# iqbal-lab-org/make_prg

Hardware: AMD Instinct MI355X
Metric: MSAs/sec (from_msa, whole node) on 30k-gene pan-genome (higher is better)
Workload: dtype u8 (+f64 KMeans)

## Files before the change

### include/mprg.h

```cpp
#ifndef MPRG_H
#define MPRG_H
#include <stdint.h>

#ifdef __cplusplus
extern "C" {
#endif

enum {
  MPRG_V_RM_BASE = 0, MPRG_V_CM_BASE = 1, MPRG_V_PITCH_C = 2, MPRG_V_PITCH_S = 3, MPRG_V_ROWS_OFF = 4,
  MPRG_V_N_ROWS = 5, MPRG_V_COL0 = 6, MPRG_V_N_COLS = 7, MPRG_V_COL_OFF = 8, MPRG_V_ROW_OFF = 9,
  MPRG_V_AUX0 = 10, MPRG_V_AUX1 = 11, MPRG_VIEW_FIELDS = 12
};
enum { MPRG_CODE_GAP = 4, MPRG_CODE_N = 11, MPRG_N_CODES = 12 };
enum { MPRG_IV_MATCH = 0, MPRG_IV_NONMATCH = 1 ,
       MPRG_IV_PURE = 2  };
enum { MPRG_ST_PARTITION_ERROR = 1, MPRG_ST_ALL_N_SLICE = 2,
       MPRG_ST_BAD_LAUNCH = 4  };
enum { MPRG_KM_RELOCATED = 1 ,
       MPRG_KM_UNSUPPORTED = 2  };

const char *mprg_version(void);
const char *mprg_last_error(void);
int mprg_device_cus(void);

// ... 53 lines not shown
int mprg_kmeans_fit_split(const int64_t *prob, const int32_t *kinfo, const int32_t *fit_list, int n_fits, int n_init,
                          const double *uniforms_dev, const double *xcounts, double *ws, int32_t *labels, double *km_info,
                          int32_t *km_status, void *stream);
int mprg_kmeans_prepare_big(const int64_t *prob, const double *xcounts, double *ws, const int32_t *list, int n_list, uint8_t *xbytes,
                            int with_tables, void *stream);
int mprg_kmeans_fit_wide(const int64_t *prob, const int32_t *kinfo, const int32_t *fit_list, int n_fits, int n_init,
                         const double *uniforms_dev, const double *xcounts, double *ws, int32_t *labels, double *km_info,
                         int32_t *km_status, const uint8_t *xbytes, void *stream);
int mprg_kmeans_wave_class(int64_t D, int64_t V, int k);
int mprg_kmeans_small_class(int64_t D, int64_t V, int k, int n_init);
int mprg_kmeans_fit_small(const int64_t *prob, const int32_t *kinfo, const int32_t *fit_list, int n_fits, int small_class, int n_init,
                          const double *uniforms_dev, const double *xcounts, double *ws, int32_t *labels, double *km_info,
                          int32_t *km_status, void *stream);
int mprg_kmeans_lds_class(int64_t D, int64_t V, int k, int n_init);
int mprg_kmeans_fit_lds(const int64_t *prob, const int32_t *kinfo, const int32_t *fit_list, int n_fits, int lds_class, int n_init,
                        const double *uniforms_dev, const double *xcounts, double *ws, int32_t *labels, double *km_info,
                        int32_t *km_status, void *stream);
int mprg_kmeans_fit_wave(const int64_t *prob, const int32_t *kinfo, const int32_t *fit_list, int n_fits, int lds_class, int n_init,
                         const double *uniforms_dev, const double *xcounts, double *ws, int32_t *labels, double *km_info,
                         int32_t *km_status, void *stream);
void mprg_random_sample_host(uint32_t seed, int n, double *out_host);

enum { MPRG_CF_TILE = 256, MPRG_CF_TILE_BIG = 32, MPRG_CF_ROWS = 1024, MPRG_CF_WIDE = 512, MPRG_CF_ROWS_WIDE = 16 };
int mprg_cluster_further(const uint8_t *arena, const int64_t *views, const int32_t *rowidx, const int64_t *prob,
                         int n_probs, int k, const int32_t *d_of_row, const int32_t *labels, int32_t *assign,
                         const int32_t *work_cols, int n_work_cols, const int32_t *work_rows, int n_work_rows,
                         int32_t *scratch, int32_t *out_further, const double *km_info, const uint8_t *gcodes, const int32_t *kinfo,
                         void *stream);
int mprg_cluster_further_bounded(const uint8_t *arena, const int64_t *views, const int32_t *rowidx, const int64_t *prob,
                                 int n_probs, int k, const int32_t *d_of_row, const int32_t *labels, int32_t *assign,
                                 const int32_t *work_cols, int n_work_cols, const int32_t *work_rows, int n_work_rows,
                                 int32_t *scratch, int32_t *out_further, const double *km_info, const uint8_t *gcodes, const int32_t *kinfo,
                                 long long max_rows, void *stream);

enum { MPRG_LOOP_GENERAL = 1, MPRG_LOOP_SMALL_LOW = 2, MPRG_LOOP_SMALL_HIGH = 4, MPRG_LOOP_SKIP_SMALL = 8,
       MPRG_LOOP_LDS = 16 ,
       MPRG_LOOP_SKIP_LDS = 32  };
int mprg_cluster_loop(const int64_t *views, const int64_t *prob, int n_probs, int n_init, const double *uniforms_dev,
                      const int32_t *uniform_offsets_host, const double *xcounts, double *ws, const int32_t *d_of_row,
                      const uint8_t *gcodes, int32_t *scratch, int32_t *labels, int32_t *assign, double *km_info, int32_t *km_status,
                      int32_t *num_clusters, int32_t *active, int64_t *stats, int forms, void *stream);

int mprg_kmeans_speculative_kinfo(const int64_t *prob, int n_probs, int n_init, int mode, const int32_t *uniform_offsets_host,
                                  long long labels_per_k, int32_t *kinfo_out, const double *ws, void *stream);

int mprg_split_children(const int64_t *views, const int32_t *rowidx, const int64_t *prob, int n_probs,
// ... 212 lines not shown
```

### make_prg_amd/csrc/k_cluster.inc

```
#define CF_TILE 256
#define CF_TILE_BIG 32
#define CF_ROWS 1024
static_assert(CF_TILE == MPRG_CF_TILE && CF_TILE_BIG == MPRG_CF_TILE_BIG && CF_ROWS == MPRG_CF_ROWS, "include/mprg.h documents the tiles");
MPRG_DEV long long cf_col_tiles(long long n_cols, long long n_rows) {
  const long long tw = n_rows > CF_ROWS ? CF_TILE_BIG : CF_TILE;
  return (n_cols + tw - 1) / tw;
}
#ifndef CFH_WIDE
#define CFH_WIDE MPRG_CF_WIDE
#endif
#define CFH_G 16
#define CFH_ROWS_WIDE 16
static_assert(CFH_ROWS_WIDE == MPRG_CF_ROWS_WIDE, "include/mprg.h documents the chunks");
MPRG_DEV int cf_chunk_rows(long long n_cols, long long n_rows) { return (n_cols >= CFH_WIDE && n_rows > CF_ROWS) ? CFH_ROWS_WIDE : CF_TILE; }
MPRG_DEV long long cf_row_chunks(long long n_cols, long long n_rows) { const int ch = cf_chunk_rows(n_cols, n_rows); return (n_rows + ch - 1) / ch; }
#define CFO_THREADS 128
#define CFO_POOL 8192
MPRG_DEV long long cf_lds_bytes(long long S, long long n, long long k) {
  const long long cp = (n + 3) & ~3LL;
  return ((S + 3) & ~3LL) + ((2 * S + 3) & ~3LL) + k * cp + S * cp;
}
MPRG_DEV bool cf_one_fits(long long S, long long n, long long k) { return S >= 1 && S < 65536 && n >= 1 && cf_lds_bytes(S, n, k) <= CFO_POOL; }
#ifndef CF_THREADS
#define CF_THREADS 128
#endif
KERNEL(k_cluster_majority, const uint8_t *arena, const int64_t *views, const int32_t *rowidx, const int64_t *prob_all,
       const int32_t *work, int k, const int32_t *d_of_row_all, const int32_t *labels_all, int32_t *assign_all,
       const double *km_info, int32_t *scratch_all, const uint8_t *gcodes_all, const int32_t *kinfo, int one_form, DsCount dc) {
  DS_GUARD(dc, 1);
  const int32_t *wk = work + 2 * (long long)BLOCK_ID;
  if (kinfo && kinfo[5 * (long long)wk[0] + 1] == 0) return;
  const int64_t *P = prob_all + (long long)wk[0] * PF;
  const ViewD d = load_view(views, (int)P[0]);
  if (one_form && cf_one_fits(d.n_rows, d.n_cols, k)) return;
  const int n = d.n_cols, S = d.n_rows, D = (int)P[1], tile = S > CF_ROWS ? CF_TILE_BIG : CF_TILE, c0 = wk[1] * tile;
  const int32_t *dor = d_of_row_all + d.row_off;
  const int32_t *labels = labels_all ? labels_all + P[10] : nullptr;
  uint8_t *maj = (uint8_t *)(scratch_all + d.col_off * 3);
  SHARED(uint32_t, cnt, 12 * CF_THREADS);
  SHARED(int32_t, first, 12 * CF_THREADS);
  if (wk[1] == 0 && labels && assign_all && (!km_info || km_info[8 * (long long)wk[0] + 3] >= (double)k)) {
    PAR_FOR(q, D) { assign_all[P[10] + q] = labels[q]; }
  }
  if (S > CF_ROWS) return;
  SHARED(int32_t, mrk, 2 * CF_ROWS);
  int32_t *mrow = mrk, *mkey = mrk + CF_ROWS;
  SHARED(int, coff, 16);
  SHARED(int, cfill, 16);
  PAR_FOR(q, 16) { coff[q] = 0; }
  BARRIER();
  PAR_FOR(i, S) {
    const int dd = dor[i];
    if (dd < 0) continue;
    const int cl = labels ? labels[dd] : 0;
    if (cl >= 0 && cl < k) ATOMIC_ADD(coff + cl + 1, 1);
  }
  BARRIER();
// ... 32 lines not shown
        for (int q = 0; q < 8; ++q) x[q] = col[(long long)mrow[m + q] * cpitch] & 15u;
#pragma unroll
        for (int q = 0; q < 8; ++q) CF_COUNT(x[q], mkey[m + q]);
      }
      for (; m < m1; ++m) { const unsigned x = col[(long long)mrow[m] * cpitch] & 15u; CF_COUNT(x, mkey[m]); }
    }
    if (slices > 1) BARRIER();
    if (live && sl == 0) {
      int best = 0; uint32_t best_n = 0; int32_t best_key = 0x7fffffff;
      for (int s = 0; s < 12; ++s) {
        uint32_t a = cnt[s * CF_THREADS + t]; int32_t key = first[s * CF_THREADS + t];
        for (int o = 1; o < slices; ++o) {
          a += cnt[s * CF_THREADS + t + o * n_items];
          const int32_t ko = first[s * CF_THREADS + t + o * n_items];
          if (ko < key) key = ko;
        }
        if (s == 0 || a > best_n || (a == best_n && key < best_key)) { best = s; best_n = a; best_key = key; }
      }
      maj[(long long)cl * n + c] = (uint8_t)best;
    }
  }
#undef CF_COUNT
}

#define CFB_THREADS 1024
KERNEL(k_cluster_majority_big, const uint8_t *arena, const int64_t *views, const int32_t *rowidx, const int64_t *prob_all,
       const int32_t *work, int k, const int32_t *d_of_row_all, const int32_t *labels_all, int32_t *scratch_all,
       const uint8_t *gcodes_all, const int32_t *kinfo, DsCount dc) {
  DS_GUARD(dc, 1);
  const int32_t *wk = work + 2 * (long long)BLOCK_ID;
  if (kinfo && kinfo[5 * (long long)wk[0] + 1] == 0) return;
  const int64_t *P = prob_all + (long long)wk[0] * PF;
  const ViewD d = load_view(views, (int)P[0]);
  const int n = d.n_cols, S = d.n_rows, c0 = wk[1] * CF_TILE_BIG;
  if (S <= CF_ROWS) return;
  const int32_t *dor = d_of_row_all + d.row_off;
  const int32_t *labels = labels_all ? labels_all + P[10] : nullptr;
  uint8_t *maj = (uint8_t *)(scratch_all + d.col_off * 3);
  __shared__ uint32_t cnt[KM_KMAX * CF_TILE_BIG * 12];
  __shared__ unsigned long long key[KM_KMAX * CF_TILE_BIG * 12];
  const int ncols = n - c0 < CF_TILE_BIG ? n - c0 : CF_TILE_BIG;
  PAR_FOR(e, k * CF_TILE_BIG * 12) { cnt[e] = 0; key[e] = ~0ULL; }
  BARRIER();
  const int t = (int)threadIdx.x, cg = t % (CF_TILE_BIG / 4), sl = t / (CF_TILE_BIG / 4), slices = N_THREADS / (CF_TILE_BIG / 4), cb = 4 * cg;
  if (cb < ncols && sl < slices) {
    const uint8_t *col = gcodes_all ? gcodes_all + d.aux0 + c0 + cb : arena + d.rm + d.col0 + c0 + cb;
    const long long cpitch = gcodes_all ? u_pitch(n) : d.pitchC;
    const int per = (S + slices - 1) / slices, i0 = sl * per, i1 = (sl + 1) * per < S ? (sl + 1) * per : S;
#define CFB_ROW(w_, dd_, i_, cl_) do {                                                                                                \
      const unsigned long long key_ = ((unsigned long long)(uint32_t)(dd_) << 32) | (uint32_t)(i_);                                   \
      _Pragma("unroll") for (int u_ = 0; u_ < 4; ++u_) {                                                                              \
        const unsigned x_ = ((w_) >> (8 * u_)) & 15u;                                                                                 \
        if (cb + u_ < ncols && x_ < 12) {                                                                                             \
          const int at_ = (((cl_) * CF_TILE_BIG + cb + u_) * 12) + (int)x_;                                                           \
// ... 15 lines not shown
    }
    for (; i < i1; ++i) {
      const int dd = dor[i];
      if (dd < 0) continue;
      const int cl = labels ? labels[dd] : 0;
      if (cl < 0 || cl >= k) continue;
      uint32_t w;
      __builtin_memcpy(&w, col + (long long)(gcodes_all ? i : view_row(d, rowidx, i)) * cpitch, 4);
      CFB_ROW(w, dd, i, cl);
    }
#undef CFB_ROW
  }
  BARRIER();
  PAR_FOR(e, k * ncols) {
    const int cl = (int)e / ncols, c = (int)e % ncols;
    const uint32_t *cn = cnt + (cl * CF_TILE_BIG + c) * 12;
    const unsigned long long *ky = key + (cl * CF_TILE_BIG + c) * 12;
    int best = 0; uint32_t best_n = 0; unsigned long long best_key = ~0ULL;
    for (int s = 0; s < 12; ++s)
      if (s == 0 || cn[s] > best_n || (cn[s] == best_n && ky[s] < best_key)) { best = s; best_n = cn[s]; best_key = ky[s]; }
    maj[(long long)cl * n + c0 + c] = (uint8_t)best;
  }
}

KERNEL(k_cluster_hamming, const uint8_t *arena, const int64_t *views, const int32_t *rowidx, const int64_t *prob_all,
       const int32_t *work, const int32_t *d_of_row_all, const int32_t *labels_all, const int32_t *scratch_all,
       int32_t *out_further, const uint8_t *gcodes_all, const int32_t *kinfo, int one_form_k, DsCount dc) {
  DS_GUARD(dc, 1);
  const int32_t *wk = work + 2 * (long long)BLOCK_ID;
  if (kinfo && kinfo[5 * (long long)wk[0] + 1] == 0) return;
  const int64_t *P = prob_all + (long long)wk[0] * PF;
  const ViewD d = load_view(views, (int)P[0]);
  if (one_form_k && cf_one_fits(d.n_rows, d.n_cols, one_form_k)) return;
  const int n = d.n_cols, S = d.n_rows, chunk = cf_chunk_rows(n, S), r0 = wk[1] * chunk;
  const int32_t *dor = d_of_row_all + d.row_off;
  const int32_t *labels = labels_all ? labels_all + P[10] : nullptr;
  const uint8_t *maj = (const uint8_t *)(scratch_all + d.col_off * 3);
  const int thresh = n < 5 ? 1 : (int)(0.2 * (double)n);
  if (gcodes_all && n >= CFH_WIDE && (N_THREADS % CFH_G) == 0) {
    const int gl = (int)threadIdx.x % CFH_G, rows_per_pass = N_THREADS / CFH_G;
    for (int ib = r0; ib < r0 + chunk && ib < S; ib += rows_per_pass) {
      const int i = ib + (int)threadIdx.x / CFH_G;
      int stop = (gl == 0) ? *(volatile int32_t *)(out_further + wk[0]) : 0;
      stop = __shfl(stop, 0, CFH_G);
      const int dd = (i < S && i < r0 + chunk) ? dor[i] : -1;
      const bool active = !stop && dd >= 0;
      const int cl = (active && labels) ? labels[dd] : 0;
      const uint8_t *m = maj + (long long)cl * n;
      const uint8_t *grow = gcodes_all + d.aux0 + (long long)(active ? i : 0) * u_pitch(n);
      int dist = 0;
      bool far = false;
      for (int c0 = 0; c0 < n; c0 += 8 * CFH_G * 4) {
        if (active && !far) {
#pragma unroll
          for (int q = 0; q < 4; ++q) {
            const int c = c0 + (q * CFH_G + gl) * 8;
// ... 29 lines not shown
    int dist = 0;
    if (gcodes_all) {
      const uint8_t *grow = gcodes_all + d.aux0 + (long long)i * u_pitch(n);
      for (int c = 0; c < n && dist <= thresh; c += 8) {
        uint64_t x, y;
        __builtin_memcpy(&x, grow + c, 8);
        __builtin_memcpy(&y, m + c, 8);
        uint64_t v = (x ^ y) & 0x0f0f0f0f0f0f0f0fULL;
        if (c + 8 > n) v &= 0xffffffffffffffffULL >> (8 * (c + 8 - n));
        const uint64_t nz = (((v & 0x7f7f7f7f7f7f7f7fULL) + 0x7f7f7f7f7f7f7f7fULL) | v) & 0x8080808080808080ULL;
        dist += __popcll(nz);
      }
    } else
    for (int c = 0; c < n && dist <= thresh; c += 8) {
      unsigned x[8], y[8];
#pragma unroll
      for (int q = 0; q < 8; ++q) { const int cc = c + q < n ? c + q : n - 1; x[q] = cell_t(arena, d, row, cc); y[q] = m[cc]; }
#pragma unroll
      for (int q = 0; q < 8; ++q) dist += (c + q < n && x[q] != y[q]) ? 1 : 0;
    }
    if (dist > thresh) out_further[wk[0]] = 1;
  }
}

#define SC_RANKS 1024
#define SC_THREADS 64
MPRG_DEV int sc_rank(const int32_t *dor, const int32_t *sor, const int32_t *assign, int kfin, int c0, int i) {
  const int c = dor[i] >= 0 ? assign[dor[i]] : kfin + sor[i];
  return c == c0 ? 0 : (c < c0 ? c + 1 : c);
}
KERNEL(k_split_children, const int64_t *views, const int32_t *rowidx, const int64_t *prob_all, const int64_t *sp_all,
       const int32_t *d_of_row_all, const int32_t *s_of_row_all, const int32_t *assign_all, int32_t *pool_out,
       int32_t *child_sizes, DsCount dc) {
  DS_GUARD(dc, 1);
  const int64_t *P = prob_all + (long long)BLOCK_ID * PF;
  const int64_t *sp = sp_all + 3 * (long long)BLOCK_ID;
  const ViewD d = load_view(views, (int)P[0]);
  const int S = d.n_rows, kfin = (int)sp[0];
  const int32_t *dor = d_of_row_all + d.row_off, *sor = s_of_row_all + d.row_off, *assign = assign_all + P[10];
  int32_t *out = pool_out + sp[1], *sizes = child_sizes + sp[2];
  const int lane = wave_lane();
  SHARED(int, off_s, SC_RANKS);
  int nshort = 0;
  for (int i = lane; i < S; i += WAVE) nshort = sor[i] + 1 > nshort ? sor[i] + 1 : nshort;
#pragma unroll
  for (int dlt = 32; dlt >= 1; dlt >>= 1) { const int y = __shfl_xor(nshort, dlt); nshort = y > nshort ? y : nshort; }
// ... 50 lines not shown
```

### make_prg_amd/csrc/k_kloop.inc

```

#ifndef KL_CF_FN
#define KL_CF_FN MPRG_DEV
#endif
#ifdef MPRG_TEST_CF_GLOBAL
#define KL_CF_IN_LDS(fits) false
#else
#define KL_CF_IN_LDS(fits) (fits)
#endif
#define KL_CF_FIELD_BITS 32
MPRG_DEV int cf_row_cluster(int i, const uint8_t *mlab_s, const int32_t *dor, const int32_t *labels) {
  if (mlab_s) return mlab_s[i];
  const int dd = dor[i];
  return dd < 0 ? 255 : labels[dd];
}
template <int FB> struct CfWords {
  static constexpr int PER = 64 / FB, W = 12 / PER;
  unsigned long long w[W];
  MPRG_DEVM void clear() {
#pragma unroll
    for (int q = 0; q < W; ++q) w[q] = 0;
  }
  MPRG_DEVM void add(unsigned x) {
    const unsigned long long inc = x < 12 ? 1ull << (FB * (x % PER)) : 0ull;
    const unsigned sel = x / PER;
// ... 91 lines not shown
    const uint8_t *m = maj + (long long)cl * n;
    const uint8_t *grow = G + (long long)i * cpitch;
    int dist = 0;
#pragma nounroll
    for (int c = 0; c < n && dist <= thresh; c += 8) {
      uint64_t x, y;
      __builtin_memcpy(&x, grow + c, 8);
      __builtin_memcpy(&y, m + c, 8);
      uint64_t v = (x ^ y) & 0x0f0f0f0f0f0f0f0fULL;
      if (c + 8 > n) v &= 0xffffffffffffffffULL >> (8 * (c + 8 - n));
      const uint64_t nz = (((v & 0x7f7f7f7f7f7f7f7fULL) + 0x7f7f7f7f7f7f7f7fULL) | v) & 0x8080808080808080ULL;
      dist += __popcll(nz);
    }
    if (dist > thresh) flag_s[0] = 1;
  }
  BARRIER();
  const bool further = flag_s[0] != 0;
  BARRIER();
  return further;
}

template <bool OPT = false>
MPRG_DEV bool cf_problem_lds(const int S, const int n, const int D, const int k, const int32_t *dor, const int32_t *labels, int32_t *assign,
                             const uint8_t *G, uint8_t *pool, int *flag_s) {
  typedef CfWords<16> Words;
  const int cpitch = u_pitch(n), cp = (n + 3) & ~3, cw4 = cp >> 2;
  uint8_t *mlab = pool;
  uint16_t *dk = (uint16_t *)(pool + ((S + 3) & ~3));
  uint8_t *majs = (uint8_t *)dk + ((2 * S + 3) & ~3);
  uint8_t *cells = majs + k * cp;
  if (!OPT || assign) { PAR_FOR(q, D) { assign[q] = labels[q]; } }
  PAR_FOR(i, S) { const int dd = dor[i]; mlab[i] = dd < 0 ? (uint8_t)255 : ((OPT && !labels) ? (uint8_t)0 : (uint8_t)labels[dd]); dk[i] = (uint16_t)dd; }
  PAR_FOR(e, S * cw4) {
    const int i = (int)((unsigned)e / (unsigned)cw4), w = (int)((unsigned)e % (unsigned)cw4);
    *(uint32_t *)(cells + i * cp + 4 * w) = *(const uint32_t *)(G + (long long)i * cpitch + 4 * w) & 0x0f0f0f0fu;
  }
  ONE_THREAD { flag_s[0] = 0; }
  BARRIER();
  PAR_FOR(item, k * n) {
    const int cl = (int)((unsigned)item / (unsigned)n), c = (int)((unsigned)item % (unsigned)n);
    Words cw;
    cw.clear();
    const uint8_t *col = cells + c;
    int i = 0;
    for (; i + 4 <= S; i += 4) {
      unsigned rc[4], x[4];
#pragma unroll
      for (int q = 0; q < 4; ++q) { rc[q] = mlab[i + q]; x[q] = col[(i + q) * cp]; }
#pragma unroll
      for (int q = 0; q < 4; ++q) cw.add(rc[q] == (unsigned)cl ? x[q] : 15u);
    }
    for (; i < S; ++i) cw.add(mlab[i] == cl ? (unsigned)col[i * cp] : 15u);
    unsigned long long best_n = 0;
#pragma unroll
    for (int s_ = 0; s_ < 12; ++s_) { const unsigned long long a = cw.count(s_); best_n = a > best_n ? a : best_n; }
    unsigned tied = 0;
#pragma unroll
    for (int s_ = 0; s_ < 12; ++s_) if (cw.count(s_) == best_n) tied |= 1u << s_;
    int best = __ffs(tied) - 1;
    if (best_n > 0 && (tied & (tied - 1))) {
      int best_key = 0x7fffffff;
// ... 185 lines not shown
      atomicAdd((unsigned long long *)stats + KL_ST_FITS, (unsigned long long)st_i[2]);
      atomicAdd((double *)stats + KL_ST_BYTES_SMALL, st_d[0]);
      if (st_d[1] != 0) atomicAdd((double *)stats + KL_ST_CF, st_d[1]);
      if (st_i[3]) stats[KL_ST_BAD] = 1;
    }
  }
}
__attribute__((amdgpu_flat_work_group_size(64, 1024), amdgpu_waves_per_eu(KM_WAVES, KM_WAVES))) __global__ void k_cluster_loop_lds(
    const int64_t *prob_all, int n_init, const double *uniforms_all, KlUoff uoff, const double *xcounts, double *ws_all,
    const int64_t *views, const int32_t *d_of_row_all, const uint8_t *gcodes_all, int32_t *scratch_all, int32_t *labels_all,
    int32_t *assign_all, double *km_info, int32_t *km_status, int32_t *num_clusters, int32_t *active, int64_t *stats, int cls, int lds_bytes,
    DsCount dc) {
  DS_GUARD(dc, 1);
  HIP_DYNAMIC_SHARED(uint8_t, pool)
  const int b = BLOCK_ID;
  if (!active[b]) return;
  const int64_t *P = prob_all + (long long)b * PF;
  const int c = kml_class_ws(P[1], P[7], num_clusters[b] + 1, n_init, true, ws_all + P[9]);
  if (c < 0 || c > cls) return;
  kll_problem(b, prob_all, n_init, uniforms_all, uoff, xcounts, ws_all, views, d_of_row_all, gcodes_all, scratch_all, labels_all, assign_all, km_info,
              km_status, num_clusters, active, stats, pool, lds_bytes, cls);
}

KERNEL(k_cluster_further_one, const int64_t *views, const int64_t *prob_all, int n_probs, int k, const int32_t *d_of_row_all,
       const int32_t *labels_all, int32_t *assign_all, const double *km_info, int32_t *out_further, const uint8_t *gcodes_all,
       const int32_t *kinfo, DsCount dc) {
  DS_GUARD(dc, 1);
  const int b = BLOCK_ID;
  if (kinfo && kinfo[5 * (long long)b + 1] == 0) return;
  const int64_t *P = prob_all + (long long)b * PF;
  const ViewD d = load_view(views, (int)P[0]);
  if (!cf_one_fits(d.n_rows, d.n_cols, k)) return;
  __shared__ __attribute__((aligned(16))) uint8_t pool[CFO_POOL];
  SHARED(int, flag, 1);
  const int32_t *labels = labels_all ? labels_all + P[10] : nullptr;
  int32_t *assign = (labels && assign_all && (!km_info || km_info[8 * (long long)b + 3] >= (double)k)) ? assign_all + P[10] : nullptr;
  const bool further = cf_problem_lds<true>(d.n_rows, d.n_cols, (int)P[1], k, d_of_row_all + d.row_off, labels, assign, gcodes_all + d.aux0, pool, flag);
  ONE_THREAD { out_further[b] = further ? 1 : 0; }
}
```

### make_prg_amd/csrc/mprg_api.hip

```cpp
#include "mprg_platform.h"
#include "../../include/mprg.h"
#include <stdio.h>
#include <initializer_list>
#include <string.h>

#include "k_ingest.inc"
#include "k_columns.inc"
#include "k_partition.inc"
#include "k_rows.inc"
#include "k_kmer.inc"
#include "k_kmeans.inc"
#include "k_kmeans_lds.inc"
#include "k_cluster.inc"
#include "k_kloop.inc"
#include "k_emit.inc"
#include "k_forest.inc"
#include "k_align.inc"
#include "k_star.inc"
#include "k_refine.inc"
#include "k_prog.inc"
#include "k_prog_band.inc"
#include "host_encoders.inc"
#include "host_batch.inc"

static thread_local char g_err[512] = "";
static int fail(const char *what) { snprintf(g_err, sizeof g_err, "%s", what); return -1; }

// ... 11 lines not shown
  const char *e = getenv(name);
  const int v = e ? atoi(e) : dflt;
  return (v >= 64 && v <= hi && v % 64 == 0) ? v : dflt;
}
static const int g_pf_threads = env_threads("MPRG_PF_THREADS", BLOCK_VIEW);
static const int g_dd_threads = env_threads("MPRG_DD_THREADS", BLOCK_VIEW, 512);
static const int g_km_threads = env_threads("MPRG_KM_THREADS", 256);
static const int g_km_wide_threads = env_threads("MPRG_KM_WIDE_THREADS", 1024);
static const int g_kp_threads = env_threads("MPRG_KP_THREADS", 0);
static const int g_kp_tiled = [] { const char *e = getenv("MPRG_KP_TILED"); return (e && atoi(e) == 0) ? 0 : 1; }();
static const int g_kpw_split = [] { const char *e = getenv("MPRG_KPW_SPLIT"); return (e && atoi(e) == 0) ? 0 : 1; }();
static const int g_kms_threads = env_threads("MPRG_KMS_THREADS", 128, 128);
static const int g_kml_flags = [] { const char *e = getenv("MPRG_KML_FLAGS"); return e ? (atoi(e) & 0x7f) : 0; }();
static const int g_kml_threads[KML_CLASSES] = {env_threads("MPRG_KML_THREADS0", 128, 256), env_threads("MPRG_KML_THREADS1", 128, 256),
                                               env_threads("MPRG_KML_THREADS2", 256, 1024), env_threads("MPRG_KML_THREADS3", 256, 1024),
                                               env_threads("MPRG_KML_THREADS4", 512, 1024), env_threads("MPRG_KML_THREADS5", 1024, 1024)};
template <class K> static int kml_raise_lds(K kernel, bool *raised, const char *what) {
  if (*raised) return 0;
  if (hipFuncSetAttribute((const void *)kernel, hipFuncAttributeMaxDynamicSharedMemorySize, KML_C5) != hipSuccess) return fail(what);
  *raised = true;
  return 0;
}
static const int g_cf_one = [] { const char *e = getenv("MPRG_CF_ONE"); return (e && atoi(e) == 0) ? 0 : 1; }();
static const int g_pw_wave = [] { const char *e = getenv("MPRG_WAVE_VIEWS"); return (e && atoi(e) == 0) ? 0 : 1; }();
static const int g_row_views = [] { const char *e = getenv("MPRG_ROW_VIEWS"); return (e && atoi(e) == 0) ? 0 : 1; }();
#define RV_THREADS 128
#define RV_THREADS_S 64

extern "C" {

#ifndef MPRG_BUILD_TAG
#define MPRG_BUILD_TAG "hip gfx950"
#endif
const char *mprg_version(void) { return "mprg 0.2 (" MPRG_BUILD_TAG ")"; }
const char *mprg_last_error(void) { return g_err; }

int mprg_device_cus(void) {
  int dev = 0; hipDeviceProp_t p;
  if (hipGetDevice(&dev) != hipSuccess || hipGetDeviceProperties(&p, dev) != hipSuccess) return fail("no HIP device");
  return p.multiProcessorCount;
}

int mprg_ingest(const uint8_t *raw, const int64_t *msa_table, int n_msas, int64_t n_tiles, const uint8_t *n_replacement,
                uint8_t *arena, int64_t arena_bytes, int32_t *status, void *stream) {
  if (n_msas <= 0) return 0;
  if (hipMemsetAsync(arena, 15, (size_t)arena_bytes, (hipStream_t)stream) != hipSuccess) return fail("memset");
// ... 318 lines not shown
int mprg_kmeans_lds_class(int64_t D, int64_t V, int k, int n_init) { return kml_class(D, V, k, n_init); }

int mprg_kmeans_fit_lds(const int64_t *prob, const int32_t *kinfo, const int32_t *fit_list, int n_fits, int lds_class, int n_init,
                        const double *uniforms_dev, const double *xcounts, double *ws, int32_t *labels, double *km_info,
                        int32_t *km_status, void *stream) {
  if (n_fits <= 0) return 0;
  if (n_init < 1 || n_init > KML_RMAX) return fail("mprg_kmeans_fit_lds: n_init must be 1..10");
  if (lds_class < 0 || lds_class >= KML_CLASSES) return fail("mprg_kmeans_fit_lds: lds_class must be 0..5 (mprg_kmeans_lds_class)");
  const int bytes = kml_class_bytes(lds_class);
  static bool raised = false;
  if (bytes > 56 * 1024 && kml_raise_lds(k_kmeans_fit_lds, &raised, "mprg_kmeans_fit_lds: the device refuses the LDS of the largest class") != 0) return -1;
  LAUNCH_LDS(k_kmeans_fit_lds, n_fits, g_kml_threads[lds_class], bytes, stream, prob, kinfo, fit_list, n_init, uniforms_dev, xcounts, ws, labels,
             km_info, km_status, bytes | (g_kml_flags << 24));
  return check_launch("k_kmeans_fit_lds");
}

int mprg_kmeans_select(const int64_t *prob, const int32_t *kinfo, int n_fits, int n_init, const double *xcounts,
                       double *ws, int32_t *labels, double *km_info, void *stream) {
  if (n_fits <= 0) return 0;
  LAUNCH(k_kmeans_select, n_fits, 256, stream, prob, kinfo, n_init, xcounts, ws, labels, km_info);
  return check_launch("k_kmeans_select");
}

static int d_cluster_further(const uint8_t *arena, const int64_t *views, const int32_t *rowidx, const int64_t *prob,
                             int n_probs, int k, const int32_t *d_of_row, const int32_t *labels, int32_t *assign,
                             const int32_t *work_cols, int n_work_cols, const int32_t *work_rows, int n_work_rows,
                             int32_t *scratch, int32_t *out_further, const double *km_info, const uint8_t *gcodes, const int32_t *kinfo,
                             void *stream, DsCount dc_cols, DsCount dc_rows, DsCount dc_probs, long long max_rows = 0);
int mprg_cluster_further(const uint8_t *arena, const int64_t *views, const int32_t *rowidx, const int64_t *prob,
                         int n_probs, int k, const int32_t *d_of_row, const int32_t *labels, int32_t *assign,
                         const int32_t *work_cols, int n_work_cols, const int32_t *work_rows, int n_work_rows,
                         int32_t *scratch, int32_t *out_further, const double *km_info, const uint8_t *gcodes, const int32_t *kinfo,
                         void *stream) {
  return d_cluster_further(arena, views, rowidx, prob, n_probs, k, d_of_row, labels, assign, work_cols, n_work_cols, work_rows, n_work_rows,
                           scratch, out_further, km_info, gcodes, kinfo, stream, DS_HOST, DS_HOST, DS_HOST);
}
int mprg_cluster_further_bounded(const uint8_t *arena, const int64_t *views, const int32_t *rowidx, const int64_t *prob,
                                 int n_probs, int k, const int32_t *d_of_row, const int32_t *labels, int32_t *assign,
                                 const int32_t *work_cols, int n_work_cols, const int32_t *work_rows, int n_work_rows,
                                 int32_t *scratch, int32_t *out_further, const double *km_info, const uint8_t *gcodes, const int32_t *kinfo,
                                 long long max_rows, void *stream) {
  return d_cluster_further(arena, views, rowidx, prob, n_probs, k, d_of_row, labels, assign, work_cols, n_work_cols, work_rows, n_work_rows,
                           scratch, out_further, km_info, gcodes, kinfo, stream, DS_HOST, DS_HOST, DS_HOST, max_rows);
}
static int d_cluster_further(const uint8_t *arena, const int64_t *views, const int32_t *rowidx, const int64_t *prob,
                             int n_probs, int k, const int32_t *d_of_row, const int32_t *labels, int32_t *assign,
                             const int32_t *work_cols, int n_work_cols, const int32_t *work_rows, int n_work_rows,
                             int32_t *scratch, int32_t *out_further, const double *km_info, const uint8_t *gcodes, const int32_t *kinfo,
                             void *stream, DsCount dc_cols, DsCount dc_rows, DsCount dc_probs, long long max_rows) {
  if (n_probs <= 0) return 0;
  if (k < 1 || k > KM_KMAX) return fail("mprg_cluster_further: k out of range");
  if (hipMemsetAsync(out_further, 0, sizeof(int32_t) * n_probs, (hipStream_t)stream) != hipSuccess) return fail("memset");
  const int one = (g_cf_one && gcodes) ? 1 : 0;
  if (one) LAUNCH(k_cluster_further_one, n_probs, CFO_THREADS, stream, views, prob, n_probs, k, d_of_row, labels, assign, km_info, out_further, gcodes,
                  kinfo, dc_probs);
  const int big = (max_rows <= 0 || max_rows > CF_ROWS) ? 1 : 0;
  LAUNCH(k_cluster_majority, n_work_cols, CF_THREADS, stream, arena, views, rowidx, prob, work_cols, k, d_of_row, labels,
         assign, km_info, scratch, gcodes, kinfo, one, dc_cols);
  if (big) LAUNCH(k_cluster_majority_big, n_work_cols, CFB_THREADS, stream, arena, views, rowidx, prob, work_cols, k, d_of_row, labels,
                  scratch, gcodes, kinfo, dc_cols);
  LAUNCH(k_cluster_hamming, n_work_rows, CF_TILE, stream, arena, views, rowidx, prob, work_rows, d_of_row, labels,
         (const int32_t *)scratch, out_further, gcodes, kinfo, one ? k : 0, dc_rows);
  return check_launch("k_cluster_further");
}

static int d_cluster_loop(const int64_t *views, const int64_t *prob, int n_probs, int n_init, const double *uniforms_dev,
                          const int32_t *uniform_offsets_host, const double *xcounts, double *ws, const int32_t *d_of_row,
                          const uint8_t *gcodes, int32_t *scratch, int32_t *labels, int32_t *assign, double *km_info, int32_t *km_status,
                          int32_t *num_clusters, int32_t *active, int64_t *stats, int forms, void *stream, DsCount dc);
int mprg_cluster_loop(const int64_t *views, const int64_t *prob, int n_probs, int n_init, const double *uniforms_dev,
                      const int32_t *uniform_offsets_host, const double *xcounts, double *ws, const int32_t *d_of_row,
                      const uint8_t *gcodes, int32_t *scratch, int32_t *labels, int32_t *assign, double *km_info, int32_t *km_status,
                      int32_t *num_clusters, int32_t *active, int64_t *stats, int forms, void *stream) {
  return d_cluster_loop(views, prob, n_probs, n_init, uniforms_dev, uniform_offsets_host, xcounts, ws, d_of_row, gcodes, scratch, labels, assign,
                        km_info, km_status, num_clusters, active, stats, forms, stream, DS_HOST);
}
static int d_cluster_loop(const int64_t *views, const int64_t *prob, int n_probs, int n_init, const double *uniforms_dev,
                          const int32_t *uniform_offsets_host, const double *xcounts, double *ws, const int32_t *d_of_row,
                          const uint8_t *gcodes, int32_t *scratch, int32_t *labels, int32_t *assign, double *km_info, int32_t *km_status,
                          int32_t *num_clusters, int32_t *active, int64_t *stats, int forms, void *stream, DsCount dc) {
  if (n_probs <= 0) return 0;
  if (n_init < 1 || n_init > KM_RMAX) return fail("n_init must be 1..16");
  if (!gcodes || !uniform_offsets_host || !stats) return fail("mprg_cluster_loop: gcodes, uniform_offsets_host and stats are required");
  if (!(forms & (7 | MPRG_LOOP_LDS))) return fail("mprg_cluster_loop: forms must name a workgroup form (MPRG_LOOP_*)");
  KlUoff uoff;
// ... 638 lines not shown
```

Baseline: 133,900.

## Bin cluster-further problems into LDS size classes with persistent compacted launches

Problems are first compacted on the device into four lists by shared-memory footprint (8K to 64K pools), and the single-block LDS path then runs once per class with per-class thread counts in persistent grid-stride loops. Problems that fit no class go to a rest list, which is handled by persistent majority/hamming kernels that ballot-scan the work list. Before, every problem got its own block and the fallback kernels early-exited. The LDS path also gains multi-slice column counting and vectorised 16-byte cell loads. The cost is an extra compaction kernel, a cached per-stream list buffer guarded by a mutex, and a raised dynamic LDS limit, which may lower occupancy for the larger classes.

After: 134,200 (median of 3 runs). About the same (+0.2%).

```diff
diff --git a/include/mprg.h b/include/mprg.h
--- a/include/mprg.h
+++ b/include/mprg.h
@@ -99,6 +99,7 @@
 void mprg_random_sample_host(uint32_t seed, int n, double *out_host);
 
 enum { MPRG_CF_TILE = 256, MPRG_CF_TILE_BIG = 32, MPRG_CF_ROWS = 1024, MPRG_CF_WIDE = 512, MPRG_CF_ROWS_WIDE = 16 };
+enum { MPRG_CF_CLASSES = 4, MPRG_CF_POOL0 = 8192 };
 int mprg_cluster_further(const uint8_t *arena, const int64_t *views, const int32_t *rowidx, const int64_t *prob,
                          int n_probs, int k, const int32_t *d_of_row, const int32_t *labels, int32_t *assign,
                          const int32_t *work_cols, int n_work_cols, const int32_t *work_rows, int n_work_rows,
diff --git a/make_prg_amd/csrc/k_cluster.inc b/make_prg_amd/csrc/k_cluster.inc
--- a/make_prg_amd/csrc/k_cluster.inc
+++ b/make_prg_amd/csrc/k_cluster.inc
@@ -14,25 +14,63 @@
 static_assert(CFH_ROWS_WIDE == MPRG_CF_ROWS_WIDE, "include/mprg.h documents the chunks");
 MPRG_DEV int cf_chunk_rows(long long n_cols, long long n_rows) { return (n_cols >= CFH_WIDE && n_rows > CF_ROWS) ? CFH_ROWS_WIDE : CF_TILE; }
 MPRG_DEV long long cf_row_chunks(long long n_cols, long long n_rows) { const int ch = cf_chunk_rows(n_cols, n_rows); return (n_rows + ch - 1) / ch; }
-#define CFO_THREADS 128
-#define CFO_POOL 8192
+#define CF_CLASSES 4
+#define CFO_POOL0 8192
+static_assert(CF_CLASSES == MPRG_CF_CLASSES && CFO_POOL0 == MPRG_CF_POOL0, "include/mprg.h documents the classes");
 MPRG_DEV long long cf_lds_bytes(long long S, long long n, long long k) {
   const long long cp = (n + 3) & ~3LL;
   return ((S + 3) & ~3LL) + ((2 * S + 3) & ~3LL) + k * cp + S * cp;
 }
-MPRG_DEV bool cf_one_fits(long long S, long long n, long long k) { return S >= 1 && S < 65536 && n >= 1 && cf_lds_bytes(S, n, k) <= CFO_POOL; }
+KML_HD int cf_class_pool(int c) { return CFO_POOL0 << c; }
+MPRG_DEV int cf_class(long long S, long long n, long long k) {
+  if (S < 1 || S >= 65536 || n < 1) return -1;
+  const long long need = cf_lds_bytes(S, n, k);
+  for (int c = 0; c < CF_CLASSES; ++c) if (need <= (long long)cf_class_pool(c)) return c;
+  return -1;
+}
+#define CFC_THREADS 256
+KERNEL(k_cf_compact, const int64_t *views, const int64_t *prob_all, int n_probs, int k, const int32_t *kinfo, int32_t *counts, int32_t *lists,
+       long long cap, int32_t *rest, DsCount dc) {
+  DS_GUARD(dc, CFC_THREADS);
+  const long long n = ds_n(dc, n_probs), b = (long long)BLOCK_ID * CFC_THREADS + (long long)threadIdx.x;
+  int li = -1;
+  if (b < n && b < cap && (!kinfo || kinfo[5 * b + 1] != 0)) {
+    const int64_t *v = views + prob_all[b * PF] * VF;
+    li = cf_class((int)v[5], (int)v[7], k);
+    if (li < 0) li = CF_CLASSES;
+  }
+  if (b < n && b < cap) rest[b] = li == CF_CLASSES ? 1 : 0;
+  const int lane = wave_lane();
+  for (int c = 0; c < CF_CLASSES; ++c) {
+    const unsigned long long m = __ballot(li == c);
+    if (m == 0) continue;
+    const int leader = __ffsll((long long)m) - 1;
+    int base = 0;
+    if (lane == leader) base = ATOMIC_ADD(counts + c, __popcll(m));
+    base = __shfl(base, leader);
+    if (li == c) lists[(long long)c * cap + base + __popcll(m & ((1ull << lane) - 1ull))] = (int32_t)b;
+  }
+}
+#define CF_REST_ITEMS(work, n_work, dc, rest, wk, ...) do {                                                                           \
+    const long long n_items_ = ds_n(dc, n_work), grid_ = (long long)gridDim.x;                                                      \
+    for (long long base_ = BLOCK_ID; base_ < n_items_; base_ += 64 * grid_) {                                                       \
+      const long long w_ = base_ + (long long)wave_lane() * grid_;                                                                  \
+      unsigned long long hits_ = __ballot(w_ < n_items_ && rest[(work)[2 * w_]] != 0);                                              \
+      while (hits_) {                                                                                                               \
+        const int32_t *wk = (work) + 2 * (base_ + (long long)(__ffsll((long long)hits_) - 1) * grid_);                              \
+        hits_ &= hits_ - 1;                                                                                                         \
+        __VA_ARGS__;                                                                                                                \
+        BARRIER();                                                                      \
+      }                                                                                                                             \
+    } } while (0)
 #ifndef CF_THREADS
 #define CF_THREADS 128
 #endif
-KERNEL(k_cluster_majority, const uint8_t *arena, const int64_t *views, const int32_t *rowidx, const int64_t *prob_all,
-       const int32_t *work, int k, const int32_t *d_of_row_all, const int32_t *labels_all, int32_t *assign_all,
-       const double *km_info, int32_t *scratch_all, const uint8_t *gcodes_all, const int32_t *kinfo, int one_form, DsCount dc) {
-  DS_GUARD(dc, 1);
-  const int32_t *wk = work + 2 * (long long)BLOCK_ID;
-  if (kinfo && kinfo[5 * (long long)wk[0] + 1] == 0) return;
+MPRG_DEV void cf_majority_item(const int32_t *wk, const uint8_t *arena, const int64_t *views, const int32_t *rowidx, const int64_t *prob_all,
+                               int k, const int32_t *d_of_row_all, const int32_t *labels_all, int32_t *assign_all,
+                               const double *km_info, int32_t *scratch_all, const uint8_t *gcodes_all) {
   const int64_t *P = prob_all + (long long)wk[0] * PF;
   const ViewD d = load_view(views, (int)P[0]);
-  if (one_form && cf_one_fits(d.n_rows, d.n_cols, k)) return;
   const int n = d.n_cols, S = d.n_rows, D = (int)P[1], tile = S > CF_ROWS ? CF_TILE_BIG : CF_TILE, c0 = wk[1] * tile;
   const int32_t *dor = d_of_row_all + d.row_off;
   const int32_t *labels = labels_all ? labels_all + P[10] : nullptr;
@@ -111,14 +149,25 @@
   }
 #undef CF_COUNT
 }
-
-#define CFB_THREADS 1024
-KERNEL(k_cluster_majority_big, const uint8_t *arena, const int64_t *views, const int32_t *rowidx, const int64_t *prob_all,
-       const int32_t *work, int k, const int32_t *d_of_row_all, const int32_t *labels_all, int32_t *scratch_all,
-       const uint8_t *gcodes_all, const int32_t *kinfo, DsCount dc) {
+KERNEL(k_cluster_majority, const uint8_t *arena, const int64_t *views, const int32_t *rowidx, const int64_t *prob_all,
+       const int32_t *work, int k, const int32_t *d_of_row_all, const int32_t *labels_all, int32_t *assign_all,
+       const double *km_info, int32_t *scratch_all, const uint8_t *gcodes_all, const int32_t *kinfo, DsCount dc) {
   DS_GUARD(dc, 1);
   const int32_t *wk = work + 2 * (long long)BLOCK_ID;
   if (kinfo && kinfo[5 * (long long)wk[0] + 1] == 0) return;
+  cf_majority_item(wk, arena, views, rowidx, prob_all, k, d_of_row_all, labels_all, assign_all, km_info, scratch_all, gcodes_all);
+}
+KERNEL(k_cluster_majority_rest, const uint8_t *arena, const int64_t *views, const int32_t *rowidx, const int64_t *prob_all,
+       const int32_t *work, int n_work, int k, const int32_t *d_of_row_all, const int32_t *labels_all, int32_t *assign_all,
+       const double *km_info, int32_t *scratch_all, const uint8_t *gcodes_all, const int32_t *rest, DsCount dc) {
+  CF_REST_ITEMS(work, n_work, dc, rest, wk,
+                cf_majority_item(wk, arena, views, rowidx, prob_all, k, d_of_row_all, labels_all, assign_all, km_info, scratch_all, gcodes_all));
+}
+
+#define CFB_THREADS 1024
+MPRG_DEV void cf_majority_big_item(const int32_t *wk, const uint8_t *arena, const int64_t *views, const int32_t *rowidx, const int64_t *prob_all,
+                                   int k, const int32_t *d_of_row_all, const int32_t *labels_all, int32_t *scratch_all,
+                                   const uint8_t *gcodes_all) {
   const int64_t *P = prob_all + (long long)wk[0] * PF;
   const ViewD d = load_view(views, (int)P[0]);
   const int n = d.n_cols, S = d.n_rows, c0 = wk[1] * CF_TILE_BIG;
@@ -180,16 +229,26 @@
     maj[(long long)cl * n + c0 + c] = (uint8_t)best;
   }
 }
-
-KERNEL(k_cluster_hamming, const uint8_t *arena, const int64_t *views, const int32_t *rowidx, const int64_t *prob_all,
-       const int32_t *work, const int32_t *d_of_row_all, const int32_t *labels_all, const int32_t *scratch_all,
-       int32_t *out_further, const uint8_t *gcodes_all, const int32_t *kinfo, int one_form_k, DsCount dc) {
+KERNEL(k_cluster_majority_big, const uint8_t *arena, const int64_t *views, const int32_t *rowidx, const int64_t *prob_all,
+       const int32_t *work, int k, const int32_t *d_of_row_all, const int32_t *labels_all, int32_t *scratch_all,
+       const uint8_t *gcodes_all, const int32_t *kinfo, DsCount dc) {
   DS_GUARD(dc, 1);
   const int32_t *wk = work + 2 * (long long)BLOCK_ID;
   if (kinfo && kinfo[5 * (long long)wk[0] + 1] == 0) return;
+  cf_majority_big_item(wk, arena, views, rowidx, prob_all, k, d_of_row_all, labels_all, scratch_all, gcodes_all);
+}
+KERNEL(k_cluster_majority_big_rest, const uint8_t *arena, const int64_t *views, const int32_t *rowidx, const int64_t *prob_all,
+       const int32_t *work, int n_work, int k, const int32_t *d_of_row_all, const int32_t *labels_all, int32_t *scratch_all,
+       const uint8_t *gcodes_all, const int32_t *rest, DsCount dc) {
+  CF_REST_ITEMS(work, n_work, dc, rest, wk,
+                cf_majority_big_item(wk, arena, views, rowidx, prob_all, k, d_of_row_all, labels_all, scratch_all, gcodes_all));
+}
+
+MPRG_DEV void cf_hamming_item(const int32_t *wk, const uint8_t *arena, const int64_t *views, const int32_t *rowidx, const int64_t *prob_all,
+                              const int32_t *d_of_row_all, const int32_t *labels_all, const int32_t *scratch_all,
+                              int32_t *out_further, const uint8_t *gcodes_all) {
   const int64_t *P = prob_all + (long long)wk[0] * PF;
   const ViewD d = load_view(views, (int)P[0]);
-  if (one_form_k && cf_one_fits(d.n_rows, d.n_cols, one_form_k)) return;
   const int n = d.n_cols, S = d.n_rows, chunk = cf_chunk_rows(n, S), r0 = wk[1] * chunk;
   const int32_t *dor = d_of_row_all + d.row_off;
   const int32_t *labels = labels_all ? labels_all + P[10] : nullptr;
@@ -265,6 +324,20 @@
     if (dist > thresh) out_further[wk[0]] = 1;
   }
 }
+KERNEL(k_cluster_hamming, const uint8_t *arena, const int64_t *views, const int32_t *rowidx, const int64_t *prob_all,
+       const int32_t *work, const int32_t *d_of_row_all, const int32_t *labels_all, const int32_t *scratch_all,
+       int32_t *out_further, const uint8_t *gcodes_all, const int32_t *kinfo, DsCount dc) {
+  DS_GUARD(dc, 1);
+  const int32_t *wk = work + 2 * (long long)BLOCK_ID;
+  if (kinfo && kinfo[5 * (long long)wk[0] + 1] == 0) return;
+  cf_hamming_item(wk, arena, views, rowidx, prob_all, d_of_row_all, labels_all, scratch_all, out_further, gcodes_all);
+}
+KERNEL(k_cluster_hamming_rest, const uint8_t *arena, const int64_t *views, const int32_t *rowidx, const int64_t *prob_all,
+       const int32_t *work, int n_work, const int32_t *d_of_row_all, const int32_t *labels_all, const int32_t *scratch_all,
+       int32_t *out_further, const uint8_t *gcodes_all, const int32_t *rest, DsCount dc) {
+  CF_REST_ITEMS(work, n_work, dc, rest, wk,
+                cf_hamming_item(wk, arena, views, rowidx, prob_all, d_of_row_all, labels_all, scratch_all, out_further, gcodes_all));
+}
 
 #define SC_RANKS 1024
 #define SC_THREADS 64
diff --git a/make_prg_amd/csrc/k_kloop.inc b/make_prg_amd/csrc/k_kloop.inc
--- a/make_prg_amd/csrc/k_kloop.inc
+++ b/make_prg_amd/csrc/k_kloop.inc
@@ -137,7 +137,7 @@
 
 template <bool OPT = false>
 MPRG_DEV bool cf_problem_lds(const int S, const int n, const int D, const int k, const int32_t *dor, const int32_t *labels, int32_t *assign,
-                             const uint8_t *G, uint8_t *pool, int *flag_s) {
+                             const uint8_t *G, uint8_t *pool, int *flag_s, const int pool_bytes = 0) {
   typedef CfWords<16> Words;
   const int cpitch = u_pitch(n), cp = (n + 3) & ~3, cw4 = cp >> 2;
   uint8_t *mlab = pool;
@@ -146,12 +146,92 @@
   uint8_t *cells = majs + k * cp;
   if (!OPT || assign) { PAR_FOR(q, D) { assign[q] = labels[q]; } }
   PAR_FOR(i, S) { const int dd = dor[i]; mlab[i] = dd < 0 ? (uint8_t)255 : ((OPT && !labels) ? (uint8_t)0 : (uint8_t)labels[dd]); dk[i] = (uint16_t)dd; }
+  if (OPT) {
+    const int g16 = cpitch >> 4, items = S * g16, nt = N_THREADS;
+    for (int e0 = MPRG_TID; e0 < items; e0 += 4 * nt) {
+      uint4 x[4];
+#pragma unroll
+      for (int q = 0; q < 4; ++q) {
+        const int e = e0 + q * nt < items ? e0 + q * nt : e0;
+        __builtin_memcpy(&x[q], G + (long long)((unsigned)e / (unsigned)g16) * cpitch + 16 * (int)((unsigned)e % (unsigned)g16), 16);
+      }
+#pragma unroll
+      for (int q = 0; q < 4; ++q) {
+        const int e = e0 + q * nt;
+        if (e >= items) break;
+        const int i = (int)((unsigned)e / (unsigned)g16), c = 16 * (int)((unsigned)e % (unsigned)g16);
+        uint32_t *to = (uint32_t *)(cells + i * cp + c);
+        if (c < cp) to[0] = x[q].x & 0x0f0f0f0fu;
+        if (c + 4 < cp) to[1] = x[q].y & 0x0f0f0f0fu;
+        if (c + 8 < cp) to[2] = x[q].z & 0x0f0f0f0fu;
+        if (c + 12 < cp) to[3] = x[q].w & 0x0f0f0f0fu;
+      }
+    }
+  } else
   PAR_FOR(e, S * cw4) {
     const int i = (int)((unsigned)e / (unsigned)cw4), w = (int)((unsigned)e % (unsigned)cw4);
     *(uint32_t *)(cells + i * cp + 4 * w) = *(const uint32_t *)(G + (long long)i * cpitch + 4 * w) & 0x0f0f0f0fu;
   }
   ONE_THREAD { flag_s[0] = 0; }
   BARRIER();
+  int slices = 1;
+  if (OPT && k * n * 2 <= N_THREADS) {
+    const long long acc_off = (cf_lds_bytes(S, n, k) + 7) & ~7LL;
+    slices = N_THREADS / (k * n);
+    if (slices > 16) slices = 16;
+    if (slices > (S + 3) / 4) slices = (S + 3) / 4;
+    if (slices > 1 && acc_off + (long long)k * n * (slices - 1) * Words::W * 8 > (long long)pool_bytes) slices = 1;
+  }
+  if (OPT && slices > 1) {
+    const int items = k * n, e = MPRG_TID;
+    unsigned long long *acc = (unsigned long long *)(pool + ((cf_lds_bytes(S, n, k) + 7) & ~7LL));
+    const bool live = e < items * slices;
+    const int item = live ? (int)((unsigned)e % (unsigned)items) : 0, sl = live ? (int)((unsigned)e / (unsigned)items) : 0;
+    const int cl = (int)((unsigned)item / (unsigned)n), c = (int)((unsigned)item % (unsigned)n);
+    Words cw;
+    cw.clear();
+    const uint8_t *col = cells + c;
+    if (live) {
+      const int per = (S + slices - 1) / slices, i1 = (sl + 1) * per < S ? (sl + 1) * per : S;
+      int i = sl * per;
+      for (; i + 4 <= i1; i += 4) {
+        unsigned rc[4], x[4];
+#pragma unroll
+        for (int q = 0; q < 4; ++q) { rc[q] = mlab[i + q]; x[q] = col[(i + q) * cp]; }
+#pragma unroll
+        for (int q = 0; q < 4; ++q) cw.add(rc[q] == (unsigned)cl ? x[q] : 15u);
+      }
+      for (; i < i1; ++i) cw.add(mlab[i] == cl ? (unsigned)col[i * cp] : 15u);
+      if (sl > 0) {
+#pragma unroll
+        for (int q = 0; q < Words::W; ++q) acc[((long long)(sl - 1) * items + item) * Words::W + q] = cw.w[q];
+      }
+    }
+    BARRIER();
+    if (live && sl == 0) {
+      for (int o = 1; o < slices; ++o)
+#pragma unroll
+        for (int q = 0; q < Words::W; ++q) cw.w[q] += acc[((long long)(o - 1) * items + item) * Words::W + q];
+    unsigned long long best_n = 0;
+#pragma unroll
+    for (int s_ = 0; s_ < 12; ++s_) { const unsigned long long a = cw.count(s_); best_n = a > best_n ? a : best_n; }
+    unsigned tied = 0;
+#pragma unroll
+    for (int s_ = 0; s_ < 12; ++s_) if (cw.count(s_) == best_n) tied |= 1u << s_;
+    int best = __ffs(tied) - 1;
+    if (best_n > 0 && (tied & (tied - 1))) {
+      int best_key = 0x7fffffff;
+#pragma nounroll
+      for (int r = 0; r < S; ++r) {
+        const unsigned x = col[r * cp];
+        if (mlab[r] != cl || !((tied >> x) & 1u)) continue;
+        const int key = (int)dk[r] * S + r;
+        if (key < best_key) { best_key = key; best = (int)x; }
+      }
+    }
+    majs[cl * cp + c] = (uint8_t)best;
+    }
+  } else
   PAR_FOR(item, k * n) {
     const int cl = (int)((unsigned)item / (unsigned)n), c = (int)((unsigned)item % (unsigned)n);
     Words cw;
@@ -383,19 +463,22 @@
               km_status, num_clusters, active, stats, pool, lds_bytes, cls);
 }
 
-KERNEL(k_cluster_further_one, const int64_t *views, const int64_t *prob_all, int n_probs, int k, const int32_t *d_of_row_all,
-       const int32_t *labels_all, int32_t *assign_all, const double *km_info, int32_t *out_further, const uint8_t *gcodes_all,
-       const int32_t *kinfo, DsCount dc) {
-  DS_GUARD(dc, 1);
-  const int b = BLOCK_ID;
-  if (kinfo && kinfo[5 * (long long)b + 1] == 0) return;
-  const int64_t *P = prob_all + (long long)b * PF;
-  const ViewD d = load_view(views, (int)P[0]);
-  if (!cf_one_fits(d.n_rows, d.n_cols, k)) return;
-  __shared__ __attribute__((aligned(16))) uint8_t pool[CFO_POOL];
+__attribute__((amdgpu_flat_work_group_size(64, 512))) __global__ void k_cluster_further_one(
+    const int64_t *views, const int64_t *prob_all, const int32_t *list, const int32_t *count, int k, int pool_bytes,
+    const int32_t *d_of_row_all, const int32_t *labels_all, int32_t *assign_all, const double *km_info, int32_t *out_further,
+    const uint8_t *gcodes_all) {
+  HIP_DYNAMIC_SHARED(unsigned long long, pool8)
   SHARED(int, flag, 1);
-  const int32_t *labels = labels_all ? labels_all + P[10] : nullptr;
-  int32_t *assign = (labels && assign_all && (!km_info || km_info[8 * (long long)b + 3] >= (double)k)) ? assign_all + P[10] : nullptr;
-  const bool further = cf_problem_lds<true>(d.n_rows, d.n_cols, (int)P[1], k, d_of_row_all + d.row_off, labels, assign, gcodes_all + d.aux0, pool, flag);
-  ONE_THREAD { out_further[b] = further ? 1 : 0; }
-}
+  const int n_list = count[0];
+  for (int i = BLOCK_ID; i < n_list; i += (int)gridDim.x) {
+    const int b = list[i];
+    const int64_t *P = prob_all + (long long)b * PF;
+    const ViewD d = load_view(views, (int)P[0]);
+    if (cf_lds_bytes(d.n_rows, d.n_cols, k) > (long long)pool_bytes) continue;
+    const int32_t *labels = labels_all ? labels_all + P[10] : nullptr;
+    int32_t *assign = (labels && assign_all && (!km_info || km_info[8 * (long long)b + 3] >= (double)k)) ? assign_all + P[10] : nullptr;
+    const bool further = cf_problem_lds<true>(d.n_rows, d.n_cols, (int)P[1], k, d_of_row_all + d.row_off, labels, assign, gcodes_all + d.aux0,
+                                              (uint8_t *)pool8, flag, pool_bytes);
+    ONE_THREAD { out_further[b] = further ? 1 : 0; }
+  }
+}
diff --git a/make_prg_amd/csrc/mprg_api.hip b/make_prg_amd/csrc/mprg_api.hip
--- a/make_prg_amd/csrc/mprg_api.hip
+++ b/make_prg_amd/csrc/mprg_api.hip
@@ -3,6 +3,8 @@
 #include <stdio.h>
 #include <initializer_list>
 #include <string.h>
+#include <mutex>
+#include <vector>
 
 #include "k_ingest.inc"
 #include "k_columns.inc"
@@ -60,6 +62,9 @@
   return 0;
 }
 static const int g_cf_one = [] { const char *e = getenv("MPRG_CF_ONE"); return (e && atoi(e) == 0) ? 0 : 1; }();
+static const int g_cfo_threads[CF_CLASSES] = {env_threads("MPRG_CFO_THREADS0", 128, 256), env_threads("MPRG_CFO_THREADS1", 256, 256),
+                                              env_threads("MPRG_CFO_THREADS2", 256, 512), env_threads("MPRG_CFO_THREADS3", 256, 512)};
+static const int g_cfo_oversub = [] { const char *e = getenv("MPRG_CFO_OVERSUB"); const int v = e ? atoi(e) : 4; return (v >= 1 && v <= 16) ? v : 4; }();
 static const int g_pw_wave = [] { const char *e = getenv("MPRG_WAVE_VIEWS"); return (e && atoi(e) == 0) ? 0 : 1; }();
 static const int g_row_views = [] { const char *e = getenv("MPRG_ROW_VIEWS"); return (e && atoi(e) == 0) ? 0 : 1; }();
 #define RV_THREADS 128
@@ -424,6 +429,37 @@
   return check_launch("k_kmeans_select");
 }
 
+#define CF_LIST_HEAD 8
+#define CF_MAX_DEVICES 64
+struct CfDevice { int id, cus; bool raised; };
+struct CfLists { int dev; hipStream_t stream; int32_t *buf; long long cap; };
+static std::mutex g_cf_mu;
+static CfDevice g_cf_devices[CF_MAX_DEVICES];
+static std::vector<CfLists> g_cf_lists;
+static CfDevice *cf_device() {
+  int id = 0;
+  if (hipGetDevice(&id) != hipSuccess || id < 0 || id >= CF_MAX_DEVICES) { fail("mprg_cluster_further: no HIP device"); return nullptr; }
+  std::lock_guard<std::mutex> g(g_cf_mu);
+  CfDevice *d = &g_cf_devices[id];
+  if (d->cus <= 0) {
+    hipDeviceProp_t p;
+    if (hipGetDeviceProperties(&p, id) != hipSuccess || p.multiProcessorCount <= 0) { fail("mprg_cluster_further: no HIP device"); return nullptr; }
+    d->id = id; d->cus = p.multiProcessorCount; d->raised = false;
+  }
+  return d;
+}
+static long long cf_lists_cap(long long n_probs) { long long cap = 1024; while (cap < n_probs) cap *= 2; return cap; }
+static int32_t *cf_lists(int dev, hipStream_t stream, long long cap) {
+  std::lock_guard<std::mutex> g(g_cf_mu);
+  CfLists *e = nullptr;
+  for (CfLists &l : g_cf_lists) if (l.dev == dev && l.stream == stream) e = &l;
+  if (e && e->cap >= cap) return e->buf;
+  void *p = nullptr;
+  if (hipMalloc(&p, sizeof(int32_t) * (size_t)(CF_LIST_HEAD + (CF_CLASSES + 1) * cap)) != hipSuccess) { fail("mprg_cluster_further: no memory for the class lists"); return nullptr; }
+  if (e) { (void)hipFree(e->buf); e->buf = (int32_t *)p; e->cap = cap; }
+  else g_cf_lists.push_back(CfLists{dev, stream, (int32_t *)p, cap});
+  return (int32_t *)p;
+}
 static int d_cluster_further(const uint8_t *arena, const int64_t *views, const int32_t *rowidx, const int64_t *prob,
                              int n_probs, int k, const int32_t *d_of_row, const int32_t *labels, int32_t *assign,
                              const int32_t *work_cols, int n_work_cols, const int32_t *work_rows, int n_work_rows,
@@ -453,16 +489,51 @@
   if (n_probs <= 0) return 0;
   if (k < 1 || k > KM_KMAX) return fail("mprg_cluster_further: k out of range");
   if (hipMemsetAsync(out_further, 0, sizeof(int32_t) * n_probs, (hipStream_t)stream) != hipSuccess) return fail("memset");
-  const int one = (g_cf_one && gcodes) ? 1 : 0;
-  if (one) LAUNCH(k_cluster_further_one, n_probs, CFO_THREADS, stream, views, prob, n_probs, k, d_of_row, labels, assign, km_info, out_further, gcodes,
-                  kinfo, dc_probs);
   const int big = (max_rows <= 0 || max_rows > CF_ROWS) ? 1 : 0;
-  LAUNCH(k_cluster_majority, n_work_cols, CF_THREADS, stream, arena, views, rowidx, prob, work_cols, k, d_of_row, labels,
-         assign, km_info, scratch, gcodes, kinfo, one, dc_cols);
-  if (big) LAUNCH(k_cluster_majority_big, n_work_cols, CFB_THREADS, stream, arena, views, rowidx, prob, work_cols, k, d_of_row, labels,
-                  scratch, gcodes, kinfo, dc_cols);
-  LAUNCH(k_cluster_hamming, n_work_rows, CF_TILE, stream, arena, views, rowidx, prob, work_rows, d_of_row, labels,
-         (const int32_t *)scratch, out_further, gcodes, kinfo, one ? k : 0, dc_rows);
+  if (!(g_cf_one && gcodes)) {
+    LAUNCH(k_cluster_majority, n_work_cols, CF_THREADS, stream, arena, views, rowidx, prob, work_cols, k, d_of_row, labels,
+           assign, km_info, scratch, gcodes, kinfo, dc_cols);
+    if (big) LAUNCH(k_cluster_majority_big, n_work_cols, CFB_THREADS, stream, arena, views, rowidx, prob, work_cols, k, d_of_row, labels,
+                    scratch, gcodes, kinfo, dc_cols);
+    LAUNCH(k_cluster_hamming, n_work_rows, CF_TILE, stream, arena, views, rowidx, prob, work_rows, d_of_row, labels,
+           (const int32_t *)scratch, out_further, gcodes, kinfo, dc_rows);
+    return check_launch("k_cluster_further");
+  }
+  CfDevice *dev = cf_device();
+  if (!dev) return -1;
+  const long long cap = cf_lists_cap(n_probs);
+  int32_t *lists = cf_lists(dev->id, (hipStream_t)stream, cap);
+  if (!lists) return -1;
+  int32_t *counts = lists, *rest = lists + CF_LIST_HEAD + (long long)CF_CLASSES * cap;
+  if (hipMemsetAsync(counts, 0, sizeof(int32_t) * CF_LIST_HEAD, (hipStream_t)stream) != hipSuccess) return fail("memset");
+  LAUNCH(k_cf_compact, (n_probs + CFC_THREADS - 1) / CFC_THREADS, CFC_THREADS, stream, views, prob, n_probs, k, kinfo, counts, lists + CF_LIST_HEAD,
+         cap, rest, dc_probs);
+  for (int c = 0; c < CF_CLASSES; ++c) {
+    const int threads = g_cfo_threads[c], pool = cf_class_pool(c);
+    if (pool > 56 * 1024 && !dev->raised) {
+      if (hipFuncSetAttribute((const void *)k_cluster_further_one, hipFuncAttributeMaxDynamicSharedMemorySize, cf_class_pool(CF_CLASSES - 1)) != hipSuccess)
+        return fail("mprg_cluster_further: the device refuses the LDS of the largest class");
+      dev->raised = true;
+    }
+    long long per_cu = (160 * 1024) / (pool + 64), by_waves = 32 / (threads / 64);
+    if (per_cu > by_waves) per_cu = by_waves;
+    long long grid = (long long)dev->cus * per_cu * g_cfo_oversub;
+    if (grid > n_probs) grid = n_probs;
+    LAUNCH_LDS(k_cluster_further_one, grid, threads, pool, stream, views, prob, (const int32_t *)(lists + CF_LIST_HEAD + (long long)c * cap),
+               (const int32_t *)(counts + c), k, pool, d_of_row, labels, assign, km_info, out_further, gcodes);
+  }
+  const long long g_cols = n_work_cols < 8LL * dev->cus ? n_work_cols : 8LL * dev->cus;
+  const long long g_rows = n_work_rows < 8LL * dev->cus ? n_work_rows : 8LL * dev->cus;
+  const long long g_big = n_work_cols < 2LL * dev->cus ? n_work_cols : 2LL * dev->cus;
+  if (n_work_cols > 0)
+    LAUNCH(k_cluster_majority_rest, g_cols, CF_THREADS, stream, arena, views, rowidx, prob, work_cols, n_work_cols, k, d_of_row, labels,
+           assign, km_info, scratch, gcodes, (const int32_t *)rest, dc_cols);
+  if (big && n_work_cols > 0)
+    LAUNCH(k_cluster_majority_big_rest, g_big, CFB_THREADS, stream, arena, views, rowidx, prob, work_cols, n_work_cols, k, d_of_row, labels,
+           scratch, gcodes, (const int32_t *)rest, dc_cols);
+  if (n_work_rows > 0)
+    LAUNCH(k_cluster_hamming_rest, g_rows, CF_TILE, stream, arena, views, rowidx, prob, work_rows, n_work_rows, d_of_row, labels,
+           (const int32_t *)scratch, out_further, gcodes, (const int32_t *)rest, dc_rows);
   return check_launch("k_cluster_further");
 }
 
```
